# LANL-Bioinformatics/KWAGE

Hardware: AMD Instinct MI355X
Metric: G k-mer·sample bit-tests/sec (+ achieved HBM GB/s of the gather kernel in `roofline`) (higher is better)
Workload: dtype u32

## Files before the change

### kwage_amd/csrc/engine.hip

```cpp
#include <hip/hip_runtime.h>
#include <hip/hip_ext.h>

#include <algorithm>
#include <chrono>
#include <cmath>
#include <cstdio>
#include <cctype>
#include <cstring>
#include <new>
#include <string>
#include <thread>
#include <vector>

#include <unistd.h>

#include "host.hpp"
#include "engine_state.hpp"
#include "kernels.hpp"

using namespace kwage;


struct TuningName { const char *name; int64_t Tuning::*field; };
static const TuningName TUNING_NAMES[] = {
	{"walk", &Tuning::walk}, {"walk_min_rows", &Tuning::walk_min_rows}, {"walk_max_kib", &Tuning::walk_max_kib}, {"walk_min_kib", &Tuning::walk_min_kib}, {"walk_tile_kib", &Tuning::walk_tile_kib},
	 {"walk_waves", &Tuning::walk_waves}, {"walk_one_wg_per_cu", &Tuning::walk_one_wg_per_cu},
	{"walk_bands", &Tuning::walk_bands}, {"walk_bands_min_gib", &Tuning::walk_bands_min_gib},
	{"and_vec", &Tuning::and_vec}, {"and_wide", &Tuning::and_wide}, {"and_wide_min_kib", &Tuning::and_wide_min_kib}, {"narrow", &Tuning::narrow}, {"force_segs", &Tuning::force_segs},
	{"ee_refine", &Tuning::ee_refine}, {"refine_seg_rows", &Tuning::refine_seg_rows}, {"refine_min_rows", &Tuning::refine_min_rows}, {"refine_max_groups", &Tuning::refine_max_groups}, {"refine_unroll", &Tuning::refine_unroll}, {"refine_list_cap", &Tuning::refine_list_cap}, {"refine_static", &Tuning::refine_static}, {"screen_wpc", &Tuning::screen_wpc}, {"count_screen_wpc", &Tuning::count_screen_wpc}, {"count_screen_min_tiles", &Tuning::count_screen_min_tiles}, {"count_screen_check", &Tuning::count_screen_check}, {"count_trunc", &Tuning::count_trunc},
	{"count_walk", &Tuning::count_walk}, {"count_walk_wpc", &Tuning::count_walk_wpc}, {"count_walk_waves", &Tuning::count_walk_waves},
	{"count_walk_min_rows", &Tuning::count_walk_min_rows},
	{"hit_sort_host", &Tuning::hit_sort_host}, {"hit_copy_piece_kb", &Tuning::hit_copy_piece_kb}, {"shared_table_log2", &Tuning::shared_table_log2},
	{"ext_launch_events", &Tuning::ext_launch_events}, {"group_contiguous", &Tuning::group_contiguous}, {"group_placement_probe", &Tuning::group_placement_probe},
};

namespace kwage {

__global__ __launch_bounds__(KM_THREADS) void kmer_kernel(KmerArgs a)
{
	extern __shared__ __attribute__((aligned(16))) unsigned long long lds_tab[];
	__shared__ uint8_t codes[KM_THREADS + KWAGE_MAX_WORD_LEN];
	__shared__ uint32_t count, tile_base;

	const uint32_t q = a.chunk_q ? a.chunk_q[blockIdx.x] : blockIdx.x;
	const uint64_t t_begin = a.chunk_q ? a.chunk_t0[blockIdx.x] : 0;
	const uint64_t s0 = a.seq_off[q];
	const uint64_t len = a.seq_off[q + 1] - s0;
	const uint64_t npos = (len >= a.k) ? (len - a.k + 1) : 0;

	if(npos == 0){
		if(threadIdx.x == 0){ a.nkmer[q] = 0; a.qthr[q] = 0; }
		return;
	}

	if(a.shared_lg){
		kmer_body<false, false>(a, q, s0, len, 0, npos, a.g_tables, a.shared_lg, codes, &count, &tile_base);
		return;
	}
	const uint32_t lg = table_log2(npos);
	if((1ull << lg) <= a.lds_slots){
		kmer_body<true, false>(a, q, s0, len, 0, npos, lds_tab, lg, codes, &count, &tile_base);
	}
	else if(npos <= KM_CHUNK){
		kmer_body<false, false>(a, q, s0, len, 0, npos, a.g_tables + a.tab_off[q], lg, codes, &count, &tile_base);
	}
	else{
		kmer_body<false, true>(a, q, s0, len, t_begin, min(npos, t_begin + (uint64_t)KM_CHUNK), a.g_tables + a.tab_off[q], lg, codes, &count, &tile_base);
	}
}

__global__ __launch_bounds__(256) void kmer_finish_kernel(KmerArgs a, uint32_t n_queries)
{
	const uint32_t q = blockIdx.x*blockDim.x + threadIdx.x;
	if(q < n_queries){ a.qthr[q] = a.complete_match ? 0u : (uint32_t)__fmul_rn(a.threshold, (float)a.nkmer[q]); }
}

__global__ __launch_bounds__(256) void remap_rows_kernel(uint32_t *rows, const uint64_t *pos_off, const uint32_t *nkmer, uint32_t num_hash,
                                                         const uint32_t *map, uint32_t map_len, unsigned long long *missing, uint32_t wgs_per_query)
{
	const uint32_t q = blockIdx.x / wgs_per_query, part = blockIdx.x % wgs_per_query;
	uint32_t *rq = rows + pos_off[q]*num_hash;
	const uint64_t n = (uint64_t)nkmer[q]*num_hash;
	for(uint64_t e = (uint64_t)part*blockDim.x + threadIdx.x; e < n; e += (uint64_t)wgs_per_query*blockDim.x){
		const uint32_t r = rq[e];
		uint32_t lo = 0, hi = map_len;
		while(lo < hi){
			const uint32_t mid = lo + (hi - lo)/2;
			if(map[mid] < r){ lo = mid + 1; } else { hi = mid; }
		}
		if(lo < map_len && map[lo] == r){ rq[e] = lo; }
		else{ rq[e] = 0; atomicAdd(missing, 1ull); }
	}
}

__global__ __launch_bounds__(SEARCH_THREADS) void and_refine_emit_kernel(SearchArgs a, RefineArgs ra)
{
	constexpr int B = 4;
	__shared__ WaveHitBuf hit_bufs[SEARCH_THREADS/WAVE];
	WaveHitBuf *hbuf = &hit_bufs[threadIdx.x >> 6];
	WaveHitState hst;
	const uint32_t lane = threadIdx.x & (WAVE - 1), l = lane & 7u, g = lane >> 3;
	const uint32_t n_clusters = refine_list_end(ra, 0);
	const uint32_t gw = __builtin_amdgcn_readfirstlane(blockIdx.x*(blockDim.x/WAVE) + (threadIdx.x >> 6));
	const uint32_t nw = gridDim.x*(blockDim.x/WAVE);
	for(uint64_t c0 = gw; c0 < n_clusters; c0 += (uint64_t)B*nw){
		RefineCluster cl[B];
		u32x4 m[B];
#pragma unroll
		for(int k = 0; k < B; ++k){
			const uint64_t ci = c0 + (uint64_t)k*nw;
			cl[k].q = REFINE_NONE;
			if(ci < n_clusters){ cl[k] = ra.clusters[ci]; }
// ... 371 lines not shown
		case 10: launch_count_nh<10>(a, s, ge); break;
		case 14: launch_count_nh<14>(a, s, ge); break;
		case 20: launch_count_nh<20>(a, s, ge); break;
		default: launch_count_nh<32>(a, s, ge); break;
	}
}

template <int PLANES, int NH, bool TRUNC>
void launch_count_walk(const SearchArgs &a, const CountWalkArgs &wa, const RefineArgs &ra, const WalkShape &w, hipStream_t s, const StageEvents &ge)
{
	if(w.lds > 48*1024){ (void)hipFuncSetAttribute((const void*)count_walk_kernel<PLANES, NH, TRUNC>, hipFuncAttributeMaxDynamicSharedMemorySize, (int)w.lds); }
	KW_GATHER_LAUNCH(ge, true, !TRUNC, (count_walk_kernel<PLANES, NH, TRUNC>), dim3(w.wgs), dim3(w.wg_waves*WAVE), w.lds, s, a, wa, ra, a.rows, a.pos_off, a.nkmer, a.qthr);
}

template <int PLANES, bool TRUNC>
void launch_count_walk_nh(const SearchArgs &a, const CountWalkArgs &wa, const RefineArgs &ra, const WalkShape &w, hipStream_t s, const StageEvents &ge)
{
	switch(a.num_hash){
		case 1: launch_count_walk<PLANES, 1, TRUNC>(a, wa, ra, w, s, ge); break;
		case 2: launch_count_walk<PLANES, 2, TRUNC>(a, wa, ra, w, s, ge); break;
		case 3: launch_count_walk<PLANES, 3, TRUNC>(a, wa, ra, w, s, ge); break;
		case 4: launch_count_walk<PLANES, 4, TRUNC>(a, wa, ra, w, s, ge); break;
		default: launch_count_walk<PLANES, 5, TRUNC>(a, wa, ra, w, s, ge); break;
	}
}

template <bool TRUNC>
void launch_count_walk_planes(uint32_t planes, const SearchArgs &a, const CountWalkArgs &wa, const RefineArgs &ra, const WalkShape &w, hipStream_t s, const StageEvents &ge)
{
	switch(planes){
		case 7: launch_count_walk_nh<TRUNC ? 10 : 7, TRUNC>(a, wa, ra, w, s, ge); break;
		case 10: launch_count_walk_nh<10, TRUNC>(a, wa, ra, w, s, ge); break;
		case 14: launch_count_walk_nh<14, TRUNC>(a, wa, ra, w, s, ge); break;
		case 20: launch_count_walk_nh<20, TRUNC>(a, wa, ra, w, s, ge); break;
		default: launch_count_walk_nh<32, TRUNC>(a, wa, ra, w, s, ge); break;
	}
}

struct RefineSetup { RefineArgs ra; uint32_t refine_wgs, emit_wgs; };

int check_refine_units(uint32_t planes, int up)
{
	if(up == 14 && planes < 14){ return fail(KWAGE_ERR_STATE, "count refine: 14-plane units with %u counter planes", planes); }
	return KWAGE_OK;
}

void launch_count_refine_and_emit(uint32_t planes, int up, const SearchArgs &a, const RefineSetup &rs, hipStream_t gs, const StageEvents &ge)
{
	const dim3 block(SEARCH_THREADS);
#define KWAGE_CR_NH(N) case N: if(up == 7){ KW_GATHER_LAUNCH(ge, false, false, (count_refine_kernel<N, 7>), dim3(rs.refine_wgs), block, 0, gs, a, rs.ra); } \
		else{ KW_GATHER_LAUNCH(ge, false, false, (count_refine_kernel<N, 14>), dim3(rs.refine_wgs), block, 0, gs, a, rs.ra); } break;
	switch(std::min(a.num_hash, 5u)){ KWAGE_CR_NH(1) KWAGE_CR_NH(2) KWAGE_CR_NH(3) KWAGE_CR_NH(4) default: KWAGE_CR_NH(5) }
#undef KWAGE_CR_NH
#define KWAGE_CE_P(P) case P: if(up == 7){ KW_GATHER_LAUNCH(ge, false, true, (count_refine_emit_kernel<P, 7>), dim3(rs.emit_wgs), block, 0, gs, a, rs.ra); } \
		else{ KW_GATHER_LAUNCH(ge, false, true, (count_refine_emit_kernel<P, (P >= 14 ? 14 : 7)>), dim3(rs.emit_wgs), block, 0, gs, a, rs.ra); } break;
	switch(planes){ KWAGE_CE_P(7) KWAGE_CE_P(10) KWAGE_CE_P(14) KWAGE_CE_P(20) default: KWAGE_CE_P(32) }
#undef KWAGE_CE_P
}

template <int PLANES>
int launch_count_combine(const SearchArgs &a, uint32_t seg_planes, hipStream_t s, const StageEvents &ge)
{
	const size_t lds = (size_t)(COMBINE_WAVES/2)*PLANES*WAVE*16;
	if(lds > 48*1024){
		HIP_TRY(hipFuncSetAttribute((const void*)count_combine_kernel<PLANES>, hipFuncAttributeMaxDynamicSharedMemorySize, (int)lds));
	}
	KW_GATHER_LAUNCH(ge, false, true, (count_combine_kernel<PLANES>), dim3((a.units_per_row + WAVE - 1)/WAVE, a.n_queries), dim3(COMBINE_WAVES*WAVE), lds, s, a, seg_planes);
	return KWAGE_OK;
}

uint64_t max_segments(const SearchArgs &a, uint64_t max_segs) { return (a.n_queries > 65535) ? 1 : max_segs; }

int reserve_zeroed(DevBuf &buf, uint64_t bytes, hipStream_t s)
{
	if(bytes <= buf.cap){ return KWAGE_OK; }
	int rc = buf.reserve(bytes);
	if(rc){ return rc; }
	HIP_TRY(hipMemsetAsync(buf.p, 0, buf.cap, s));
	return KWAGE_OK;
}

int refine_setup(Slot *sl, const Tuning &tn, const SearchArgs &a, uint64_t total_rows, uint64_t max_rows, uint32_t max_seg, uint64_t item_bytes, uint64_t unit_bytes,
                 uint64_t tiles, uint64_t screen_waves, uint64_t ncu, hipStream_t gs, RefineSetup *out,
                 uint64_t exact_clusters = 0, uint64_t exact_items = 0, uint64_t exact_units = 0)
{
	int rc;
	RefineArgs &ra = out->ra;
	ra.seg_rows = (uint32_t)std::min<int64_t>(std::max<int64_t>(tn.refine_seg_rows, 8), max_seg);
	ra.seg_rows = (uint32_t)std::max<uint64_t>(ra.seg_rows, (max_rows + 65535)/65536);
	ra.min_rows = (uint32_t)std::max<int64_t>(tn.refine_min_rows, 1);
	ra.max_groups = (uint32_t)std::min<int64_t>(std::max<int64_t>(tn.refine_max_groups, 0), 16);
	uint64_t items = std::min<uint64_t>(std::max<uint64_t>(8ull*a.n_queries, 1u << 16), 1u << 20);
	items = std::max<uint64_t>(std::min<uint64_t>(items, (256ull << 20)/item_bytes), 1024);
	uint64_t units = std::min<uint64_t>(std::max<uint64_t>(32*total_rows/ra.seg_rows, 1u << 18), 1u << 25);
	if(unit_bytes){ units = std::max<uint64_t>(std::min<uint64_t>(units, (512ull << 20)/unit_bytes), 4096); }
	if(tn.refine_list_cap > 0){ items = units = (uint64_t)std::min<int64_t>(tn.refine_list_cap, 1 << 20); }
	uint64_t clusters = items;
	if(exact_units){ clusters = exact_clusters; items = exact_items; units = exact_units; }
	if(exact_units && tn.refine_list_cap > 0){ clusters = items = units = (uint64_t)std::min<int64_t>(tn.refine_list_cap, 1 << 20); }
	const uint64_t tiles_per_wave = (tiles + screen_waves - 1)/std::max<uint64_t>(screen_waves, 1);
	auto list = [&](uint64_t cap, uint64_t stat_max, uint64_t chunk_max) {
		RefineList ls;
		ls.cap = (uint32_t)cap;
		ls.stat = (tn.refine_static && !exact_units) ? (uint32_t)std::min<uint64_t>(stat_max, cap/2/std::max<uint64_t>(screen_waves, 1)) : 0u;
		ls.base = (uint32_t)(ls.stat*screen_waves);
		ls.chunk = exact_units ? 1u : (uint32_t)std::max<uint64_t>(1, std::min<uint64_t>(chunk_max, tiles_per_wave/4));
		return ls;
	};
	ra.lc = list(clusters, 32, 32);
	ra.li = list(items, 64, 64);
	ra.lu = list(units, 256, 256);
	if((rc = sl->ref_counters.reserve(8*sizeof(uint32_t)))){ return rc; }
	if((rc = sl->ref_clusters.reserve(clusters*sizeof(RefineCluster)))){ return rc; }
	if((rc = sl->ref_masks.reserve(items*item_bytes))){ return rc; }
	if((rc = sl->ref_units.reserve(units*sizeof(RefineUnit)))){ return rc; }
	if(unit_bytes && (rc = sl->ref_slab.reserve(units*unit_bytes))){ return rc; }
	ra.counters = (uint32_t*)sl->ref_counters.p;
	ra.clusters = (RefineCluster*)sl->ref_clusters.p;
	ra.masks = (uint32_t*)sl->ref_masks.p;
	ra.units = (RefineUnit*)sl->ref_units.p;
	ra.slab = (uint32_t*)sl->ref_slab.p;
	HIP_TRY(hipMemsetAsync(ra.counters, 0, 8*sizeof(uint32_t), gs));
	sl->ref_base[0] = ra.lc.base; sl->ref_base[1] = ra.li.base; sl->ref_base[2] = ra.lu.base;
	sl->ref_cap[0] = ra.lc.cap; sl->ref_cap[1] = ra.li.cap; sl->ref_cap[2] = ra.lu.cap;
	ra.queue_batch = (uint32_t)std::max<uint64_t>(1, std::min<uint64_t>(16, tiles/(8*std::max<uint64_t>(screen_waves, 1))));
	ra.check_every = (tn.count_screen_check == 16 || tn.count_screen_check == 32 || tn.count_screen_check == 64) ? (uint32_t)tn.count_screen_check : 8u;
	out->refine_wgs = (uint32_t)(ncu*8);
	out->emit_wgs = (uint32_t)(ncu*4);
	return KWAGE_OK;
}

uint32_t count_screen_blocks_per_cu(uint32_t planes, uint32_t nh)
{
	static int cache[3][5] = {};
	const int pi = (planes <= 7) ? 0 : (planes <= 10) ? 1 : 2, ni = (int)std::min(std::max(nh, 1u), 5u) - 1;
	if(cache[pi][ni] == 0){
		int nb = 0;
		hipError_t e = hipErrorUnknown;
#define KWAGE_OCC_NH(P, N) case N: e = hipOccupancyMaxActiveBlocksPerMultiprocessor(&nb, count_screen_kernel<P, N>, SEARCH_THREADS, 0); break;
#define KWAGE_OCC_P(I, P) case I: switch(ni + 1){ KWAGE_OCC_NH(P, 1) KWAGE_OCC_NH(P, 2) KWAGE_OCC_NH(P, 3) KWAGE_OCC_NH(P, 4) default: KWAGE_OCC_NH(P, 5) } break;
		switch(pi){ KWAGE_OCC_P(0, 7) KWAGE_OCC_P(1, 10) default: KWAGE_OCC_P(2, 14) }
#undef KWAGE_OCC_P
#undef KWAGE_OCC_NH
		if(e != hipSuccess || nb <= 0){ (void)hipGetLastError(); nb = 2; }
		cache[pi][ni] = nb;
	}
	return (uint32_t)cache[pi][ni];
}

int launch_search_stage(Slot *sl, kwage_group *g, kwage_batch *b, const KmerLayout *L, float threshold, uint32_t flags,
                        kwage_hit *d_hits, uint64_t cap, unsigned long long *hit_count, hipStream_t gs, const StageEvents &ge)
{
	const Tuning &tn = g->ctx->tune;
	const uint64_t ncu = (uint64_t)std::max(g->ctx->ncu, 1);
	SearchArgs a;
	a.db = g->d_bits;
	a.stride = g->stride;
	a.units_per_row = (uint32_t)(g->stride/16);
	a.valid = g->d_valid;
	a.rows = (const uint32_t*)sl->rows.p;
	a.pos_off = L->d_pos_off;
	a.nkmer = sl->d_nkmer;
	a.qthr = sl->d_qthr;
	a.num_hash = g->params.num_hash;
	a.n_queries = b->n;
	a.hits = d_hits;
	a.cap = cap;
	a.hit_count = hit_count;
	a.early_exit = (flags & KWAGE_SEARCH_EARLY_EXIT) ? 1 : 0;
	a.partial = nullptr;
	a.col_base = sl->col_base;
	a.runs = sl->n_runs ? (unsigned long long*)sl->runs.p : nullptr;
	a.runs_per_query = sl->runs_per_query;
	int rc;

	if(threshold == 1.0f){
		const uint64_t wide_tiles = (uint64_t)a.n_queries*((a.units_per_row + 4*WAVE - 1)/(4*WAVE));
		const bool wide_ok = tn.and_wide && !(flags & KWAGE_SEARCH_EARLY_EXIT) && wide_tiles >= 8*ncu;
		const bool wide_rows = wide_ok && a.units_per_row > (uint32_t)std::max<int64_t>(tn.and_wide_min_kib, 1)*WAVE;
		const AndCfg cfg = and_config(tn, a.units_per_row, wide_rows);
		a.chunks = (a.units_per_row + WAVE*cfg.vec - 1)/(WAVE*cfg.vec);
		choose_segments(a, L->max_pos, max_segments(a, 4096), tn.force_segs);
		if((uint64_t)a.n_queries*a.segs*a.chunks/4 + 1 > 0x7FFFFFFFull){ return fail(KWAGE_ERR_ARG, "batch too large for one launch"); }
		if(tn.narrow && a.segs == 1 && a.units_per_row <= 32 && a.n_queries >= 64){
			const uint32_t G = (a.units_per_row <= 4) ? 16 : (a.units_per_row <= 8) ? 8 : (a.units_per_row <= 16) ? 4 : 2;
			const uint64_t waves = ((uint64_t)a.n_queries + G - 1)/G;
			const dim3 grid((uint32_t)((waves + 3)/4)), block(SEARCH_THREADS);
			const int unroll = (waves < ncu*16) ? 16 : 8;
			snprintf(sl->kernel_name, sizeof(sl->kernel_name), "and_narrow_kernel<%u,%d>", G, unroll);
#define KWAGE_NARROW_CASE(GG) case GG: \
				if(unroll == 16){ KW_GATHER_LAUNCH(ge, true, true, (and_narrow_kernel<GG, 16>), grid, block, 0, gs, a); } \
				else{ KW_GATHER_LAUNCH(ge, true, true, (and_narrow_kernel<GG, 8>), grid, block, 0, gs, a); } break;
			switch(G){
				KWAGE_NARROW_CASE(16) KWAGE_NARROW_CASE(8) KWAGE_NARROW_CASE(4)
				default: KWAGE_NARROW_CASE(2)
			}
#undef KWAGE_NARROW_CASE
			HIP_TRY(hipGetLastError());
			return KWAGE_OK;
		}
		if(a.early_exit && tn.ee_refine && a.units_per_row >= WAVE && tn.force_segs <= 0){
			RefineSetup rs;
			const int vec = (a.units_per_row >= 4*WAVE) ? 2 : 1;
			a.segs = 1;
			a.chunks = (a.units_per_row + WAVE*vec - 1)/(WAVE*vec);
			const uint64_t tiles = (uint64_t)a.n_queries*a.chunks;
			const uint64_t screen_waves = (std::min<uint64_t>(tiles, ncu*(uint64_t)std::max<int64_t>(tn.screen_wpc, 1)) + 3)/4*4;
			if((rc = refine_setup(sl, tn, a, L->total_pos*a.num_hash, L->max_pos*a.num_hash, 1u << 20, 128, 0, tiles, screen_waves, ncu, gs, &rs))){ return rc; }
			const int unroll = (tn.refine_unroll == 16) ? 16 : 8;
			snprintf(sl->kernel_name, sizeof(sl->kernel_name), "and_screen_kernel<%d,8>+refine<%d>", vec, unroll);
			const dim3 grid((uint32_t)(screen_waves/4)), block(SEARCH_THREADS);
			if(vec == 2){ KW_GATHER_LAUNCH(ge, true, false, (and_screen_kernel<2, 8>), grid, block, 0, gs, a, rs.ra); }
			else{ KW_GATHER_LAUNCH(ge, true, false, (and_screen_kernel<1, 8>), grid, block, 0, gs, a, rs.ra); }
			if(unroll == 16){ KW_GATHER_LAUNCH(ge, false, false, (and_refine_kernel<16>), dim3(rs.refine_wgs), block, 0, gs, a, rs.ra); }
			else{ KW_GATHER_LAUNCH(ge, false, false, (and_refine_kernel<8>), dim3(rs.refine_wgs), block, 0, gs, a, rs.ra); }
			KW_GATHER_LAUNCH(ge, false, true, and_refine_emit_kernel, dim3(rs.emit_wgs), block, 0, gs, a, rs.ra);
			HIP_TRY(hipGetLastError());
			return KWAGE_OK;
		}
		const int walk_knob = (int)tn.walk;
		const uint64_t walk_min_rows = (tn.walk_min_rows >= 0) ? (uint64_t)tn.walk_min_rows : (uint64_t)WALK_MIN_ROWS_PER_WAVE*256*WALK_WAVES_PER_CU;
		const uint32_t kib = (a.units_per_row + WAVE - 1)/WAVE;
		const uint32_t walk_max_kib = (uint32_t)std::max<int64_t>(tn.walk_max_kib, 0);
		const uint32_t walk_tile = (uint32_t)std::min<int64_t>(std::max<int64_t>(tn.walk_tile_kib, 1), 16);
		const uint32_t coltiles = (kib + walk_tile - 1)/walk_tile, walk_ch = (kib + coltiles - 1)/coltiles;
		const bool walk_ee_ok = !a.early_exit;
		const uint64_t walk_slots = (uint64_t)coltiles*L->total_pos;
		const uint32_t walk_min_kib = (uint32_t)std::max<int64_t>(tn.walk_min_kib, 1);
		const int walk_unroll = (walk_ch <= 2) ? 8 : 4;
		if(walk_knob && walk_ee_ok && kib >= walk_min_kib && kib <= walk_max_kib && walk_slots*a.num_hash >= walk_min_rows && walk_slots > 0){
			const uint64_t chip_waves = ncu*WALK_WAVES_PER_CU;
			const uint64_t want_waves = (tn.walk_waves > 0) ? std::min<uint64_t>((uint64_t)tn.walk_waves, walk_slots)
				: std::max<uint64_t>(1, std::min<uint64_t>(chip_waves, walk_slots*a.num_hash/WALK_MIN_ROWS_PER_WAVE));
			const WalkShape shape = walk_shape(tn, want_waves, ncu);
			const uint32_t wgs = shape.wgs;
			const uint64_t waves = (uint64_t)wgs*shape.wg_waves;
			const uint64_t band_items = L->total_pos*a.num_hash;
			const bool big_enough = g->alloc_bytes >= ((uint64_t)std::max<int64_t>(tn.walk_bands_min_gib, 0) << 30);
			const uint32_t bands = !big_enough ? 0u : (tn.walk_bands < 0) ? (g->mixes_regions ? 3u : 0u) : (uint32_t)std::min<int64_t>(tn.walk_bands, BAND_MAX);
			if(bands >= 2 && coltiles == 1 && walk_ch >= 3 &&
			   (uint64_t)a.n_queries*16*1024 <= (256ull << 20) && band_items < 0x7FFFFFFFull){
				BandArgs ba;
				ba.bands = bands;
				ba.rows_per_band = (uint32_t)((g->nrows + bands - 1)/bands);
				if((rc = sl->band_rows.reserve(band_items*sizeof(uint32_t)))){ return rc; }
				if((rc = sl->band_loc.reserve((uint64_t)a.n_queries*(bands + 1)*sizeof(uint32_t)))){ return rc; }
				if((rc = reserve_zeroed(sl->band_or, (uint64_t)a.n_queries*16*1024, gs))){ return rc; }
				if((rc = reserve_zeroed(sl->band_state, (uint64_t)a.n_queries*sizeof(uint32_t), gs))){ return rc; }
				ba.orbuf = (uint32_t*)sl->band_or.p;
				ba.state = (uint32_t*)sl->band_state.p;
				uint32_t *loc = (uint32_t*)sl->band_loc.p, *rows2 = (uint32_t*)sl->band_rows.p;
				KW_GATHER_LAUNCH(ge, true, false, band_bucket_kernel, dim3(a.n_queries), dim3(256), 0, gs, a.rows, a.pos_off, a.nkmer, a.num_hash,
				                 ba.bands, ba.rows_per_band, loc, rows2);
				WalkArgs wb;
				wb.total_slots = walk_slots;
				wb.per_wave = (walk_slots + waves - 1)/waves;
				wb.coltiles = 1;
				wb.orbuf = nullptr; wb.done = nullptr;
				a.segs = 1;
				a.chunks = 1;
				snprintf(sl->kernel_name, sizeof(sl->kernel_name), "and_band_walk_kernel<%u,4>", walk_ch);
				const dim3 grid(wgs), block(shape.wg_waves*WAVE), fgrid((a.n_queries + 3)/4);
#define KWAGE_BAND_LAUNCH(CH, U) do { \
					if(shape.lds > 48*1024){ (void)hipFuncSetAttribute((const void*)and_band_walk_kernel<CH, U>, hipFuncAttributeMaxDynamicSharedMemorySize, (int)shape.lds); } \
					KW_GATHER_LAUNCH(ge, false, false, (and_band_walk_kernel<CH, U>), grid, block, shape.lds, gs, a, ba, wb, (const uint32_t*)rows2, (const uint32_t*)loc, a.pos_off, a.nkmer); \
					KW_GATHER_LAUNCH(ge, false, true, (and_band_finish_kernel<CH>), fgrid, dim3(256), 0, gs, a, ba, a.nkmer); } while(0)
#define KWAGE_BAND_CASE(CH) case CH: \
					KWAGE_BAND_LAUNCH(CH, 4); break;
				switch(walk_ch){
					KWAGE_BAND_CASE(3) KWAGE_BAND_CASE(4) KWAGE_BAND_CASE(5) KWAGE_BAND_CASE(6) KWAGE_BAND_CASE(7)
					KWAGE_BAND_CASE(8) KWAGE_BAND_CASE(9) KWAGE_BAND_CASE(10) KWAGE_BAND_CASE(11) KWAGE_BAND_CASE(12)
					KWAGE_BAND_CASE(13) KWAGE_BAND_CASE(14) KWAGE_BAND_CASE(15)
					default: KWAGE_BAND_CASE(16)
				}
#undef KWAGE_BAND_CASE
#undef KWAGE_BAND_LAUNCH
				HIP_TRY(hipGetLastError());
				return KWAGE_OK;
			}
			WalkArgs wa;
			wa.total_slots = walk_slots;
			wa.per_wave = (walk_slots + waves - 1)/waves;
			wa.coltiles = coltiles;
			if((rc = reserve_zeroed(sl->walk_or, waves*16*1024, gs))){ return rc; }
			if((rc = reserve_zeroed(sl->walk_done, waves*2*sizeof(uint32_t), gs))){ return rc; }
			wa.orbuf = (uint32_t*)sl->walk_or.p;
			wa.done = (uint32_t*)sl->walk_done.p;
			a.segs = 1;
			a.chunks = coltiles;
			snprintf(sl->kernel_name, sizeof(sl->kernel_name), "and_walk_kernel<%u,%d>", walk_ch, walk_unroll);
			const dim3 grid(wgs), block(shape.wg_waves*WAVE);
#define KWAGE_WALK_LAUNCH(...) do { \
				if(shape.lds > 48*1024){ (void)hipFuncSetAttribute((const void*)and_walk_kernel<__VA_ARGS__>, hipFuncAttributeMaxDynamicSharedMemorySize, (int)shape.lds); } \
				KW_GATHER_LAUNCH(ge, true, true, (and_walk_kernel<__VA_ARGS__>), grid, block, shape.lds, gs, a, wa, a.rows, a.pos_off, a.nkmer); } while(0)
#define KWAGE_WALK_CASE(CH) case CH: KWAGE_WALK_LAUNCH(CH, 4); break;
#define KWAGE_WALK_CASE8(CH) case CH: KWAGE_WALK_LAUNCH(CH, 8); break;
// ... 1076 lines not shown
```

### kwage_amd/csrc/engine_state.hpp

```cpp
#ifndef KWAGE_AMD_ENGINE_STATE_HPP
#define KWAGE_AMD_ENGINE_STATE_HPP

#include <hip/hip_runtime.h>

#include <algorithm>
#include <deque>
#include <memory>
#include <mutex>
#include <vector>

#include "internal.h"

#define HIP_TRY(expr)                                                                          \
	do {                                                                                       \
		hipError_t _e = (expr);                                                                \
		if(_e != hipSuccess){                                                                  \
			return fail(KWAGE_ERR_DEVICE, "%s failed: %s (%s:%d)", #expr, hipGetErrorString(_e), \
			            __FILE__, __LINE__);                                                   \
		}                                                                                      \
	} while(0)

struct kwage_group;
struct kwage_batch;
struct kwage_ctx;
// ... 149 lines not shown
	{
		if(!b.p){ return; }
		{
			std::lock_guard<std::mutex> lock(mu);
			uint64_t held = 0;
			for(const PinBuf &c : cached){ held += c.cap; }
			if(open && cached.size() < MAX_CACHED_BLOCKS && held + b.cap <= MAX_CACHED_BYTES){
				cached.push_back(b);
				b.p = nullptr; b.cap = 0;
				return;
			}
		}
		b.release();
	}
	void close()
	{
		std::lock_guard<std::mutex> lock(mu);
		open = false;
		for(PinBuf &c : cached){ c.release(); }
		cached.clear();
	}
};


struct Slot {
	hipStream_t stream = nullptr;
	hipEvent_t ev[4] = {nullptr, nullptr, nullptr, nullptr};
	hipEvent_t kmer_done = nullptr;
	hipEvent_t gather_done = nullptr;
	DevBuf rows, tables, partial;
	DevBuf result;
	uint64_t *d_counters = nullptr;
	uint32_t *d_nkmer = nullptr, *d_qthr = nullptr;
	kwage_hit *d_hits = nullptr;
	uint64_t hit_cap = 0, head_bytes = 0;
	PinBuf h_stage;
	DevBuf sort_scratch;
	DevBuf runs;
	uint64_t n_runs = 0;
	uint32_t runs_per_query = 0;
	bool busy = false;
	kwage_group *g = nullptr;
	kwage_batch *b = nullptr;
	const KmerLayout *lay = nullptr;
	float threshold = 1.0f;
	uint32_t flags = 0;
	uint32_t launches = 0;
	char kernel_name[64] = "";
	DevBuf walk_or, walk_done;
	DevBuf band_rows, band_loc, band_or, band_state;
	DevBuf cwalk_slab, cwalk_arrived;
	DevBuf ref_counters, ref_clusters, ref_masks, ref_units, ref_slab;
	DevBuf trunc_dev;
	PinBuf trunc_host;
	uint32_t ref_base[3] = {0, 0, 0}, ref_cap[3] = {0, 0, 0};
	uint64_t staged_hits = 0;
	kwage_hit *ext_hits = nullptr;
	uint64_t ext_cap = 0;
	uint64_t *ext_count = nullptr;
	bool append = false, append_reset = false;
	uint32_t col_base = 0;
};

struct Tuning {
	int64_t walk = 4;
	int64_t walk_min_rows = -1;
	int64_t walk_max_kib = 16;
	int64_t walk_tile_kib = 16;
	int64_t walk_min_kib = 2;
	int64_t walk_waves = 0;
	int64_t walk_one_wg_per_cu = 1;
	int64_t walk_bands = -1;
	int64_t walk_bands_min_gib = 48;
	int64_t and_vec = 0;
	int64_t and_wide_min_kib = 16;
	int64_t and_wide = 1;
	int64_t narrow = 1;
	int64_t force_segs = 0;
	int64_t ee_refine = 1;
	int64_t refine_seg_rows = 32;
	int64_t refine_min_rows = 32;
	int64_t refine_max_groups = 4;
	int64_t refine_unroll = 8;
	int64_t screen_wpc = 20;
	int64_t count_screen_wpc = 32;
	int64_t count_screen_min_tiles = 8192;
	int64_t count_trunc = 1;
	int64_t count_screen_check = 8;
	int64_t refine_static = 1;
	int64_t refine_list_cap = 0;
	int64_t count_walk = 1;
	int64_t count_walk_wpc = 8;
	int64_t count_walk_waves = 0;
	int64_t count_walk_min_rows = -1;
	int64_t hit_sort_host = 0;
	int64_t hit_copy_piece_kb = 0;
	int64_t ext_launch_events = 1;
	int64_t shared_table_log2 = 0;
	int64_t group_contiguous = 1;
	int64_t group_placement_probe = 1;
};

}

struct kwage_ctx {
	int device = -1;
	int ncu = 0;
	kwage::Tuning tune;
	hipStream_t stream = nullptr;
	hipStream_t gather_stream = nullptr;
	hipStream_t upload_stream = nullptr;
	kwage::Slot slot[2];
	kwage::DevBuf kmers;
	kwage::DevPool batch_pool;
	kwage::PinBuf load_pin[2];
	kwage::DevBuf load_dev[3];
	hipEvent_t load_done[3] = {nullptr, nullptr, nullptr};
	void *map_base = nullptr;
	size_t map_len = 0;
	hipEvent_t map_done = nullptr;
	struct LockedWindow { void *base; size_t len; hipEvent_t done; bool owns_event; };
	std::deque<LockedWindow> locked;
	std::vector<hipEvent_t> spare_events;
	volatile uint64_t *load_progress = nullptr;
	std::shared_ptr<kwage::PinnedPool> result_pool = std::make_shared<kwage::PinnedPool>();
	std::vector<int> numa_cpus;
	int numa_node = -1;
};

struct kwage_group {
	kwage_ctx *ctx = nullptr;
	kwage_params params{};
	uint64_t nrows = 0;
	uint64_t stride = 0;
	uint64_t next_byte = 0;
	uint64_t num_columns = 0;
	uint8_t *d_bits = nullptr;
	uint8_t *d_valid = nullptr;
	uint64_t alloc_bytes = 0;
	uint32_t placement_candidates = 0;
	double placement_kept_gbps = 0, placement_other_gbps = 0;
	double placement_windowed_gbps = 0;
	bool mixes_regions = false;
	std::vector<uint8_t> h_valid;
	bool finalized = false;
	double density = 0.25;
	double density_max = 1.0;
	std::vector<uint32_t> h_row_map;
	uint32_t *d_row_map = nullptr;
};

namespace kwage {

struct KmerLayout {
	uint32_t k = 0;
	uint64_t total_pos = 0;
	uint64_t max_pos = 0;
	uint64_t table_slots = 0;
	uint64_t *d_pos_off = nullptr;
	uint64_t *d_tab_off = nullptr;
	uint32_t *d_chunk_q = nullptr;
	uint64_t *d_chunk_t0 = nullptr;
	uint64_t n_chunks = 0;
	bool multi_chunk = false;
	std::vector<uint64_t> h_pos_off;
	DevPool *pool = nullptr;
// ... 68 lines not shown
```

### kwage_amd/csrc/kernels.hpp

```cpp
#ifndef KWAGE_AMD_KERNELS_HPP
#define KWAGE_AMD_KERNELS_HPP

#include <hip/hip_runtime.h>
#include <stdint.h>

#include "kwage_amd.h"
#include "kmer_device.hpp"

namespace kwage {

static constexpr int WAVE = 64;
static constexpr int KM_THREADS = 256;
static constexpr uint32_t KM_LDS_SLOTS = 4096;
static constexpr uint32_t KM_CHUNK = 1024;
static constexpr uint64_t KM_EMPTY = ~0ull;
static constexpr int SEARCH_THREADS = 256;


__device__ __forceinline__ uint32_t table_log2(uint64_t npos)
{
	uint32_t lg = 6;
	while((1ull << lg) < 2*npos){ ++lg; }
	return lg;
}
// ... 334 lines not shown
		if(k0 >= k1){ return; }
	}
	const uint32_t nrows = (k1 - k0)*a.num_hash;
	const uint32_t *rq = a.rows + (a.pos_off[q] + k0)*a.num_hash;

	uint32_t unit[VEC];
	bool live[VEC];
	u32x4 acc[VEC];
#pragma unroll
	for(int v = 0; v < VEC; ++v){
		const uint32_t u = c*(WAVE*VEC) + v*WAVE + lane;
		live[v] = (u < a.units_per_row);
		unit[v] = live[v] ? u : (a.units_per_row - 1);
		acc[v] = ~(u32x4)(0u);
	}

	uint32_t i = 0;
	bool dead = false;
	for(; i + UNROLL <= nrows; i += UNROLL){
		u32x4 x[UNROLL][VEC];
#pragma unroll
		for(int u = 0; u < UNROLL; ++u){
			const uint32_t r = rq[i + u];
			const u32x4 *p = reinterpret_cast<const u32x4*>(a.db + (uint64_t)r*a.stride);
#pragma unroll
			for(int v = 0; v < VEC; ++v){ x[u][v] = load16<NT>(p + unit[v]); }
		}
#pragma unroll
		for(int u = 0; u < UNROLL; ++u){
#pragma unroll
			for(int v = 0; v < VEC; ++v){ acc[v] &= x[u][v]; }
		}
		if(a.early_exit){
			bool nz = false;
#pragma unroll
			for(int v = 0; v < VEC; ++v){ nz |= ((acc[v].x | acc[v].y | acc[v].z | acc[v].w) != 0); }
			if(!__any(nz)){ dead = true; break; }
		}
	}
	for(; !dead && i < nrows; ++i){
		const uint32_t r = rq[i];
		const u32x4 *p = reinterpret_cast<const u32x4*>(a.db + (uint64_t)r*a.stride);
#pragma unroll
		for(int v = 0; v < VEC; ++v){ acc[v] &= load16<NT>(p + unit[v]); }
	}

#pragma unroll
	for(int v = 0; v < VEC; ++v){
		if(SEG){
			if(live[v]){
				uint32_t *m = a.partial + ((uint64_t)q*a.units_per_row + unit[v])*4;
#pragma unroll
				for(int d = 0; d < 4; ++d){
					if(acc[v][d] != ~0u){ atomicAnd(m + d, acc[v][d]); }
				}
			}
		}
		else{
			emit_mask_hits(a, q, unit[v], acc[v], n, (uint64_t)q*a.runs_per_query + c*VEC + v, live[v]);
		}
	}
}

struct RefineUnit { uint32_t item, r0, r1, unit0, rq_lo, rq_hi, q, pad; };
struct RefineCluster {
	uint32_t q, kstep_groups, first_item, n;
	uint32_t first_unit, nseg, pad0, pad1;
};
static constexpr uint32_t REFINE_NONE = 0xFFFFFFFFu;

struct RefineList { uint32_t cap, stat, base, chunk; };
struct RefineArgs {
	uint32_t *counters;
	RefineCluster *clusters;
	uint32_t *masks;
	RefineUnit *units;
	uint32_t *slab;
	RefineList lc, li, lu;
	uint32_t seg_rows;
	uint32_t min_rows;
	uint32_t max_groups;
	uint32_t queue_batch;
	uint32_t check_every;
};

__device__ __forceinline__ uint32_t group_bits(uint64_t lanes)
{
	uint32_t g = 0;
#pragma unroll
	for(int k = 0; k < 8; ++k){ g |= ((lanes >> (8*k)) & 0xFFull) ? (1u << k) : 0u; }
	return g;
}

__device__ __forceinline__ uint32_t nth_set_bit(uint32_t bits, uint32_t j)
{
	for(uint32_t k = 0; k < j; ++k){ bits &= bits - 1; }
	return __ffs(bits) - 1;
}

struct RefineChunk { uint32_t next = 0, end = 0; };

__device__ __forceinline__ void refine_none_clusters(const RefineArgs &ra, uint32_t from, uint32_t to)
{
	to = min(to, ra.lc.cap);
	for(uint32_t i = from + (threadIdx.x & (WAVE - 1)); i < to; i += WAVE){ ra.clusters[i].q = REFINE_NONE; }
}
__device__ __forceinline__ void refine_none_units(const RefineArgs &ra, uint32_t from, uint32_t to)
{
	to = min(to, ra.lu.cap);
	for(uint32_t i = from + (threadIdx.x & (WAVE - 1)); i < to; i += WAVE){ ra.units[i].item = REFINE_NONE; }
}

__device__ __forceinline__ uint32_t refine_take(const RefineArgs &ra, int which, RefineChunk &ch, uint32_t need)
{
	const RefineList &ls = (which == 0) ? ra.lc : (which == 1) ? ra.li : ra.lu;
	if(ch.end - ch.next < need){
		if(which == 0){ refine_none_clusters(ra, ch.next, ch.end); } else if(which == 2){ refine_none_units(ra, ch.next, ch.end); }
		ch.next = ch.end = 0;
		if((uint64_t)ls.base + __hip_atomic_load(ra.counters + which, __ATOMIC_RELAXED, __HIP_MEMORY_SCOPE_AGENT) >= ls.cap){ return REFINE_NONE; }
		const uint32_t want = max(need, ls.chunk);
		uint32_t r = 0;
		if((threadIdx.x & (WAVE - 1)) == 0){ r = atomicAdd(ra.counters + which, want); }
		const uint64_t at = (uint64_t)ls.base + __builtin_amdgcn_readfirstlane(r);
		if(at + want > ls.cap){
			if(at < ls.cap){
				if(which == 0){ refine_none_clusters(ra, (uint32_t)at, ls.cap); } else if(which == 2){ refine_none_units(ra, (uint32_t)at, ls.cap); }
			}
			return REFINE_NONE;
		}
		ch.next = (uint32_t)at;
		ch.end = (uint32_t)at + want;
	}
	const uint32_t at = ch.next;
	ch.next += need;
	return at;
}

__device__ __forceinline__ uint32_t refine_list_end(const RefineArgs &ra, int which)
{
	const RefineList &ls = (which == 0) ? ra.lc : (which == 1) ? ra.li : ra.lu;
	return (uint32_t)min((uint64_t)ls.base + ra.counters[which], (uint64_t)ls.cap);
}

template <int VEC, int UNROLL>
__global__ __launch_bounds__(SEARCH_THREADS) void and_screen_kernel(SearchArgs a, RefineArgs ra)
{
	const uint32_t lane = threadIdx.x & (WAVE - 1);
	const uint64_t n_tiles = (uint64_t)a.n_queries*a.chunks;
	const uint32_t n_waves = gridDim.x*(blockDim.x/WAVE);
	const uint32_t gw = __builtin_amdgcn_readfirstlane(blockIdx.x*(blockDim.x/WAVE) + (threadIdx.x >> 6));
	__shared__ WaveHitBuf hit_bufs[SEARCH_THREADS/WAVE];
	WaveHitBuf *hbuf = &hit_bufs[threadIdx.x >> 6];
	WaveHitState hst;
	RefineChunk cc, ci, cu;
	cc.next = gw*ra.lc.stat; cc.end = cc.next + ra.lc.stat;
	ci.next = gw*ra.li.stat; ci.end = ci.next + ra.li.stat;
	cu.next = gw*ra.lu.stat; cu.end = cu.next + ra.lu.stat;
	bool lists_full = false;
	for(uint64_t tile = gw; tile < n_tiles; tile += n_waves){
		const uint32_t q = __builtin_amdgcn_readfirstlane((uint32_t)(tile / a.chunks));
		const uint32_t c = __builtin_amdgcn_readfirstlane((uint32_t)(tile % a.chunks));
		const uint32_t n = a.nkmer[q];
		if(n == 0){ continue; }
		const uint32_t nrows = n*a.num_hash;
		const uint64_t rq_off = a.pos_off[q]*a.num_hash;
		const uint32_t *rq = a.rows + rq_off;

		uint32_t unit[VEC];
		u32x4 acc[VEC];
#pragma unroll
		for(int v = 0; v < VEC; ++v){
			const uint32_t u = c*(WAVE*VEC) + v*WAVE + lane;
			const bool live = (u < a.units_per_row);
			unit[v] = live ? u : (a.units_per_row - 1);
			acc[v] = live ? reinterpret_cast<const u32x4*>(a.valid)[u] : (u32x4)(0u);
		}

		bool may_hand_over = !lists_full, gone = false;
		uint32_t i = 0;
		for(; i + UNROLL <= nrows; i += UNROLL){
			u32x4 x[UNROLL][VEC];
#pragma unroll
			for(int u = 0; u < UNROLL; ++u){
				const uint32_t r = rq[i + u];
				const u32x4 *p = reinterpret_cast<const u32x4*>(a.db + (uint64_t)r*a.stride);
#pragma unroll
				for(int v = 0; v < VEC; ++v){ x[u][v] = load16<true>(p + unit[v]); }
			}
#pragma unroll
			for(int u = 0; u < UNROLL; ++u){
#pragma unroll
				for(int v = 0; v < VEC; ++v){ acc[v] &= x[u][v]; }
			}
			uint32_t gb[VEC], ngroups = 0;
#pragma unroll
			for(int v = 0; v < VEC; ++v){
				gb[v] = group_bits(__ballot((acc[v].x | acc[v].y | acc[v].z | acc[v].w) != 0));
				ngroups += __popc(gb[v]);
			}
			if(ngroups == 0){ gone = true; break; }
			const uint32_t done = i + UNROLL;
			if(may_hand_over && ngroups <= ra.max_groups && nrows - done >= ra.min_rows && (done >= 2*UNROLL || nrows < 4*ra.seg_rows)){
				may_hand_over = false;
				const uint32_t nseg = (nrows - done + ra.seg_rows - 1)/ra.seg_rows;
				uint32_t nc = 0;
#pragma unroll
				for(int v = 0; v < VEC; ++v){ nc += gb[v] ? 1u : 0u; }
				const uint32_t nu = ngroups*nseg;
				const uint32_t c0 = refine_take(ra, 0, cc, nc);
				const uint32_t i0 = (c0 != REFINE_NONE) ? refine_take(ra, 1, ci, ngroups) : REFINE_NONE;
				const uint32_t u0 = (i0 != REFINE_NONE) ? refine_take(ra, 2, cu, nu) : REFINE_NONE;
				if(u0 == REFINE_NONE){
					if(c0 != REFINE_NONE){ refine_none_clusters(ra, c0, c0 + nc); }
					lists_full = true;
					continue;
				}
				uint32_t cidx = c0, ii = i0, all_groups = 0;
#pragma unroll
				for(int v = 0; v < VEC; ++v){
					all_groups |= gb[v] << (8*v);
					if(!gb[v]){ continue; }
					if(lane == 0){
						RefineCluster cl; cl.q = q; cl.kstep_groups = ((c*VEC + v) << 8) | gb[v]; cl.first_item = ii; cl.n = n;
						cl.first_unit = 0; cl.nseg = 0; cl.pad0 = 0; cl.pad1 = 0;
						ra.clusters[cidx] = cl;
					}
					const uint32_t k = lane >> 3;
					if((gb[v] >> k) & 1u){
						const uint32_t it = ii + __popc(gb[v] & ((1u << k) - 1u));
						reinterpret_cast<u32x4*>(ra.masks)[(uint64_t)it*8 + (lane & 7u)] = acc[v];
					}
					++cidx;
					ii += __popc(gb[v]);
				}
				for(uint32_t e = lane; e < nu; e += WAVE){
					const uint32_t j = e / nseg, sg = e % nseg;
					const uint32_t gpos = nth_set_bit(all_groups, j);
					RefineUnit un;
					un.item = i0 + j;
					un.r0 = done + sg*ra.seg_rows;
					un.r1 = min(nrows, un.r0 + ra.seg_rows);
					un.unit0 = c*(WAVE*VEC) + gpos*8u;
					un.rq_lo = (uint32_t)rq_off; un.rq_hi = (uint32_t)(rq_off >> 32);
					un.q = q; un.pad = 0;
					ra.units[u0 + e] = un;
				}
				gone = true;
				break;
			}
		}
		if(gone){ continue; }
		for(; i < nrows; ++i){
			const uint32_t r = rq[i];
			const u32x4 *p = reinterpret_cast<const u32x4*>(a.db + (uint64_t)r*a.stride);
#pragma unroll
			for(int v = 0; v < VEC; ++v){ acc[v] &= load16<true>(p + unit[v]); }
		}
#pragma unroll
		for(int v = 0; v < VEC; ++v){
			emit_masked_hits_buffered(a, hbuf, hst, q, unit[v], acc[v], n, (uint64_t)q*a.runs_per_query + c*VEC + v);
		}
	}
	wave_hits_flush(a, hbuf, hst);
	refine_none_clusters(ra, cc.next, cc.end);
	refine_none_units(ra, cu.next, cu.end);
}

template <int UNROLL>
__global__ __launch_bounds__(SEARCH_THREADS) void and_refine_kernel(SearchArgs a, RefineArgs ra)
{
	static_assert(UNROLL == 8 || UNROLL == 16, "eight or sixteen rows in flight");
	const uint32_t lane = threadIdx.x & (WAVE - 1), l = lane & 7u, sh = lane & ~7u;
	const uint32_t n_units = refine_list_end(ra, 2);
	const uint64_t gw = (uint64_t)blockIdx.x*(blockDim.x/WAVE) + (threadIdx.x >> 6);
	const uint64_t step = (uint64_t)gridDim.x*(blockDim.x/WAVE)*8;
	for(uint64_t base = gw*8; base < n_units; base += step){
		const uint64_t u = base + (lane >> 3);
		RefineUnit un;
		un.item = REFINE_NONE;
		if(u < n_units){ un = ra.units[u]; }
		bool on = (un.item != REFINE_NONE);
		uint32_t *M = ra.masks;
		u32x4 m = (u32x4)(0u);
		if(on){
			M = ra.masks + ((uint64_t)un.item*8 + l)*4;
#pragma unroll
			for(int d = 0; d < 4; ++d){ m[d] = __hip_atomic_load(M + d, __ATOMIC_RELAXED, __HIP_MEMORY_SCOPE_AGENT); }
		}
		on = on && (((uint32_t)(__ballot((m.x | m.y | m.z | m.w) != 0) >> sh) & 0xFFu) != 0);
		if(on){
			const uint32_t *rq = a.rows + (((uint64_t)un.rq_hi << 32) | un.rq_lo);
			const u32x4 *col = reinterpret_cast<const u32x4*>(a.db) + (un.unit0 + l);
			u32x4 acc = ~(u32x4)(0u);
			bool alive = true;
			for(uint32_t b = un.r0; alive && b < un.r1; b += 64){
				uint32_t idx[8];
#pragma unroll
				for(int k = 0; k < 8; ++k){ idx[k] = rq[min(b + 8u*k + l, un.r1 - 1)]; }
#pragma unroll
				for(int k = 0; k < 8; k += UNROLL/8){
					if(b + 8u*k >= un.r1){ break; }
					u32x4 x[UNROLL];
#pragma unroll
					for(int j = 0; j < UNROLL; ++j){
						const uint32_t r = __shfl(idx[k + j/8], sh + (j & 7));
						x[j] = load16<true>(reinterpret_cast<const u32x4*>(reinterpret_cast<const uint8_t*>(col) + (uint64_t)r*a.stride));
					}
#pragma unroll
					for(int j = 0; j < UNROLL; ++j){ acc &= x[j]; }
					if((((uint32_t)(__ballot((acc.x | acc.y | acc.z | acc.w) != 0) >> sh)) & 0xFFu) == 0){ alive = false; break; }
				}
			}
#pragma unroll
			for(int d = 0; d < 4; ++d){
				if(m[d] & ~acc[d]){ __hip_atomic_fetch_and(M + d, acc[d], __ATOMIC_RELAXED, __HIP_MEMORY_SCOPE_AGENT); }
			}
		}
	}
}


static constexpr int WALK_WG_WAVES = 8;
static constexpr uint32_t WALK_DEAD = 1u;
static constexpr uint32_t WALK_DIRTY = 2u;

struct WalkArgs {
	uint64_t total_slots;
	uint64_t per_wave;
	uint32_t coltiles;
	uint32_t *orbuf;
	uint32_t *done;
};

template <int CH, int UNROLL>
__global__ __launch_bounds__(WALK_WG_WAVES*WAVE) __attribute__((amdgpu_waves_per_eu(2, 2))) void and_walk_kernel(SearchArgs a, WalkArgs wa, const uint32_t *__restrict__ rows,
// ... 1026 lines not shown
```

Measured before the change: 52170.

## Add in-wave narrow refinement in AND screen kernel and skip refine lists when small

When only a few 8-lane groups of a tile remain live and few rows are left, the screen kernel now finishes those groups itself. Each wave splits the remaining rows across its lanes, loads many rows in flight per lane, and combines results with cross-lane AND reductions, instead of handing work to the separate refine and emit kernels. If every query's row count fits under the in-wave threshold, the refine lists are sized to zero and the refine and emit launches are skipped entirely. This removes list-management atomics, extra kernel launches and the underused tail loop. In exchange the serialized per-group loop can leave a wave running long on tiles with many rows.

```diff
diff --git a/kwage_amd/csrc/engine.hip b/kwage_amd/csrc/engine.hip
--- a/kwage_amd/csrc/engine.hip
+++ b/kwage_amd/csrc/engine.hip
@@ -27,7 +27,7 @@
 	 {"walk_waves", &Tuning::walk_waves}, {"walk_one_wg_per_cu", &Tuning::walk_one_wg_per_cu},
 	{"walk_bands", &Tuning::walk_bands}, {"walk_bands_min_gib", &Tuning::walk_bands_min_gib},
 	{"and_vec", &Tuning::and_vec}, {"and_wide", &Tuning::and_wide}, {"and_wide_min_kib", &Tuning::and_wide_min_kib}, {"narrow", &Tuning::narrow}, {"force_segs", &Tuning::force_segs},
-	{"ee_refine", &Tuning::ee_refine}, {"refine_seg_rows", &Tuning::refine_seg_rows}, {"refine_min_rows", &Tuning::refine_min_rows}, {"refine_max_groups", &Tuning::refine_max_groups}, {"refine_unroll", &Tuning::refine_unroll}, {"refine_list_cap", &Tuning::refine_list_cap}, {"refine_static", &Tuning::refine_static}, {"screen_wpc", &Tuning::screen_wpc}, {"count_screen_wpc", &Tuning::count_screen_wpc}, {"count_screen_min_tiles", &Tuning::count_screen_min_tiles}, {"count_screen_check", &Tuning::count_screen_check}, {"count_trunc", &Tuning::count_trunc},
+	{"ee_refine", &Tuning::ee_refine}, {"refine_seg_rows", &Tuning::refine_seg_rows}, {"refine_min_rows", &Tuning::refine_min_rows}, {"refine_max_groups", &Tuning::refine_max_groups}, {"refine_unroll", &Tuning::refine_unroll}, {"refine_inwave_rows", &Tuning::refine_inwave_rows}, {"refine_inwave_first", &Tuning::refine_inwave_first}, {"refine_inwave_fallback", &Tuning::refine_inwave_fallback},{"refine_list_cap", &Tuning::refine_list_cap}, {"refine_static", &Tuning::refine_static}, {"screen_wpc", &Tuning::screen_wpc}, {"count_screen_wpc", &Tuning::count_screen_wpc}, {"count_screen_min_tiles", &Tuning::count_screen_min_tiles}, {"count_screen_check", &Tuning::count_screen_check}, {"count_trunc", &Tuning::count_trunc},
 	{"count_walk", &Tuning::count_walk}, {"count_walk_wpc", &Tuning::count_walk_wpc}, {"count_walk_waves", &Tuning::count_walk_waves},
 	{"count_walk_min_rows", &Tuning::count_walk_min_rows},
 	{"hit_sort_host", &Tuning::hit_sort_host}, {"hit_copy_piece_kb", &Tuning::hit_copy_piece_kb}, {"shared_table_log2", &Tuning::shared_table_log2},
@@ -565,7 +565,7 @@
 
 int refine_setup(Slot *sl, const Tuning &tn, const SearchArgs &a, uint64_t total_rows, uint64_t max_rows, uint32_t max_seg, uint64_t item_bytes, uint64_t unit_bytes,
                  uint64_t tiles, uint64_t screen_waves, uint64_t ncu, hipStream_t gs, RefineSetup *out,
-                 uint64_t exact_clusters = 0, uint64_t exact_items = 0, uint64_t exact_units = 0)
+                 uint64_t exact_clusters = 0, uint64_t exact_items = 0, uint64_t exact_units = 0, bool no_lists = false)
 {
 	int rc;
 	RefineArgs &ra = out->ra;
@@ -581,6 +581,7 @@
 	uint64_t clusters = items;
 	if(exact_units){ clusters = exact_clusters; items = exact_items; units = exact_units; }
 	if(exact_units && tn.refine_list_cap > 0){ clusters = items = units = (uint64_t)std::min<int64_t>(tn.refine_list_cap, 1 << 20); }
+	if(no_lists){ clusters = items = units = 0; }
 	const uint64_t tiles_per_wave = (tiles + screen_waves - 1)/std::max<uint64_t>(screen_waves, 1);
 	auto list = [&](uint64_t cap, uint64_t stat_max, uint64_t chunk_max) {
 		RefineList ls;
@@ -593,7 +594,7 @@
 	ra.lc = list(clusters, 32, 32);
 	ra.li = list(items, 64, 64);
 	ra.lu = list(units, 256, 256);
-	if((rc = sl->ref_counters.reserve(8*sizeof(uint32_t)))){ return rc; }
+	if((rc = reserve_zeroed(sl->ref_counters, 8*sizeof(uint32_t), gs))){ return rc; }
 	if((rc = sl->ref_clusters.reserve(clusters*sizeof(RefineCluster)))){ return rc; }
 	if((rc = sl->ref_masks.reserve(items*item_bytes))){ return rc; }
 	if((rc = sl->ref_units.reserve(units*sizeof(RefineUnit)))){ return rc; }
@@ -603,10 +604,12 @@
 	ra.masks = (uint32_t*)sl->ref_masks.p;
 	ra.units = (RefineUnit*)sl->ref_units.p;
 	ra.slab = (uint32_t*)sl->ref_slab.p;
-	HIP_TRY(hipMemsetAsync(ra.counters, 0, 8*sizeof(uint32_t), gs));
+	if(!no_lists){ HIP_TRY(hipMemsetAsync(ra.counters, 0, 8*sizeof(uint32_t), gs)); }
 	sl->ref_base[0] = ra.lc.base; sl->ref_base[1] = ra.li.base; sl->ref_base[2] = ra.lu.base;
 	sl->ref_cap[0] = ra.lc.cap; sl->ref_cap[1] = ra.li.cap; sl->ref_cap[2] = ra.lu.cap;
 	ra.queue_batch = (uint32_t)std::max<uint64_t>(1, std::min<uint64_t>(16, tiles/(8*std::max<uint64_t>(screen_waves, 1))));
+	ra.inwave_rows = 0;
+	ra.inwave_flags = 0;
 	ra.check_every = (tn.count_screen_check == 16 || tn.count_screen_check == 32 || tn.count_screen_check == 64) ? (uint32_t)tn.count_screen_check : 8u;
 	out->refine_wgs = (uint32_t)(ncu*8);
 	out->emit_wgs = (uint32_t)(ncu*4);
@@ -689,12 +692,20 @@
 			a.chunks = (a.units_per_row + WAVE*vec - 1)/(WAVE*vec);
 			const uint64_t tiles = (uint64_t)a.n_queries*a.chunks;
 			const uint64_t screen_waves = (std::min<uint64_t>(tiles, ncu*(uint64_t)std::max<int64_t>(tn.screen_wpc, 1)) + 3)/4*4;
-			if((rc = refine_setup(sl, tn, a, L->total_pos*a.num_hash, L->max_pos*a.num_hash, 1u << 20, 128, 0, tiles, screen_waves, ncu, gs, &rs))){ return rc; }
+			const uint64_t inwave_rows = (uint64_t)std::min<int64_t>(std::max<int64_t>(tn.refine_inwave_rows, 0), 0xFFFFFFFFll);
+			const bool screen_only = inwave_rows > 0 && L->max_pos*a.num_hash <= inwave_rows;
+			if((rc = refine_setup(sl, tn, a, L->total_pos*a.num_hash, L->max_pos*a.num_hash, 1u << 20, 128, 0, tiles, screen_waves, ncu, gs, &rs, 0, 0, 0, screen_only))){ return rc; }
+			rs.ra.inwave_rows = (uint32_t)inwave_rows;
+			rs.ra.inwave_flags = (tn.refine_inwave_first ? INWAVE_FIRST : 0u) | (tn.refine_inwave_fallback ? INWAVE_FALLBACK : 0u);
 			const int unroll = (tn.refine_unroll == 16) ? 16 : 8;
 			snprintf(sl->kernel_name, sizeof(sl->kernel_name), "and_screen_kernel<%d,8>+refine<%d>", vec, unroll);
 			const dim3 grid((uint32_t)(screen_waves/4)), block(SEARCH_THREADS);
-			if(vec == 2){ KW_GATHER_LAUNCH(ge, true, false, (and_screen_kernel<2, 8>), grid, block, 0, gs, a, rs.ra); }
-			else{ KW_GATHER_LAUNCH(ge, true, false, (and_screen_kernel<1, 8>), grid, block, 0, gs, a, rs.ra); }
+			if(vec == 2){ KW_GATHER_LAUNCH(ge, true, screen_only, (and_screen_kernel<2, 8>), grid, block, 0, gs, a, rs.ra); }
+			else{ KW_GATHER_LAUNCH(ge, true, screen_only, (and_screen_kernel<1, 8>), grid, block, 0, gs, a, rs.ra); }
+			if(screen_only){
+				HIP_TRY(hipGetLastError());
+				return KWAGE_OK;
+			}
 			if(unroll == 16){ KW_GATHER_LAUNCH(ge, false, false, (and_refine_kernel<16>), dim3(rs.refine_wgs), block, 0, gs, a, rs.ra); }
 			else{ KW_GATHER_LAUNCH(ge, false, false, (and_refine_kernel<8>), dim3(rs.refine_wgs), block, 0, gs, a, rs.ra); }
 			KW_GATHER_LAUNCH(ge, false, true, and_refine_emit_kernel, dim3(rs.emit_wgs), block, 0, gs, a, rs.ra);
diff --git a/kwage_amd/csrc/engine_state.hpp b/kwage_amd/csrc/engine_state.hpp
--- a/kwage_amd/csrc/engine_state.hpp
+++ b/kwage_amd/csrc/engine_state.hpp
@@ -255,6 +255,9 @@
 	int64_t refine_min_rows = 32;
 	int64_t refine_max_groups = 4;
 	int64_t refine_unroll = 8;
+	int64_t refine_inwave_rows = 1024;
+	int64_t refine_inwave_first = 1;
+	int64_t refine_inwave_fallback = 1;
 	int64_t screen_wpc = 20;
 	int64_t count_screen_wpc = 32;
 	int64_t count_screen_min_tiles = 8192;
diff --git a/kwage_amd/csrc/kernels.hpp b/kwage_amd/csrc/kernels.hpp
--- a/kwage_amd/csrc/kernels.hpp
+++ b/kwage_amd/csrc/kernels.hpp
@@ -440,7 +440,12 @@
 	uint32_t max_groups;
 	uint32_t queue_batch;
 	uint32_t check_every;
+	uint32_t inwave_rows;
+	uint32_t inwave_flags;
 };
+static constexpr uint32_t INWAVE_FIRST = 1u;
+static constexpr uint32_t INWAVE_FALLBACK = 2u;
+static constexpr int INWAVE_LOADS = 8;
 
 __device__ __forceinline__ uint32_t group_bits(uint64_t lanes)
 {
@@ -498,6 +503,53 @@
 {
 	const RefineList &ls = (which == 0) ? ra.lc : (which == 1) ? ra.li : ra.lu;
 	return (uint32_t)min((uint64_t)ls.base + ra.counters[which], (uint64_t)ls.cap);
+}
+
+template <int D, int T>
+__device__ __forceinline__ void and_inwave_loads(const uint8_t *col, uint64_t stride, const uint32_t (&idx)[D/8], u32x4 (&x)[D])
+{
+	if constexpr(T < D){
+		const uint32_t r = (uint32_t)__builtin_amdgcn_ds_swizzle((int)idx[T >> 3], 0x18 | ((T & 7) << 5));
+		x[T] = load16<true>(reinterpret_cast<const u32x4*>(col + (uint64_t)r*stride));
+		and_inwave_loads<D, T + 1>(col, stride, idx, x);
+	}
+}
+
+template <int D>
+__device__ __forceinline__ u32x4 and_inwave_group(const SearchArgs &a, const uint32_t *rq, uint32_t r0, uint32_t nrows, uint32_t unit0, u32x4 gm)
+{
+	static_assert(D == 8 || D == 16, "eight or sixteen rows in flight per lane");
+	constexpr int NI = D/8;
+	uint32_t lane = threadIdx.x & (WAVE - 1);
+	asm volatile("" : "+v"(lane));
+	const uint32_t l = lane & 7u;
+	const u32x4 *col = reinterpret_cast<const u32x4*>(a.db) + min(unit0 + l, a.units_per_row - 1);
+	uint32_t idx[NI];
+#pragma unroll
+	for(int k = 0; k < NI; ++k){ idx[k] = rq[min(r0 + 64u*k + lane, nrows - 1)]; }
+	for(uint32_t b = r0; b < nrows; b += 8u*D){
+		u32x4 x[D];
+		and_inwave_loads<D, 0>(reinterpret_cast<const uint8_t*>(col), a.stride, idx, x);
+		uint32_t nxt[NI];
+#pragma unroll
+		for(int k = 0; k < NI; ++k){ nxt[k] = rq[min(b + 8u*D + 64u*k + lane, nrows - 1)]; }
+		u32x4 p = x[0];
+#pragma unroll
+		for(int t = 1; t < D; ++t){ p &= x[t]; }
+#pragma unroll
+		for(int d = 8; d < WAVE; d <<= 1){
+#pragma unroll
+			for(int e = 0; e < 4; ++e){ p[e] &= __shfl_xor(p[e], d); }
+		}
+		gm &= p;
+#pragma unroll
+		for(int k = 0; k < NI; ++k){
+			asm volatile("" : "+v"(nxt[k]));
+			idx[k] = nxt[k];
+		}
+		if(!__any((gm.x | gm.y | gm.z | gm.w) != 0)){ break; }
+	}
+	return gm;
 }
 
 template <int VEC, int UNROLL>
@@ -534,7 +586,7 @@
 			acc[v] = live ? reinterpret_cast<const u32x4*>(a.valid)[u] : (u32x4)(0u);
 		}
 
-		bool may_hand_over = !lists_full, gone = false;
+		bool may_hand_over = !lists_full, gone = false, narrowed = false;
 		uint32_t i = 0;
 		for(; i + UNROLL <= nrows; i += UNROLL){
 			u32x4 x[UNROLL][VEC];
@@ -558,6 +610,23 @@
 			}
 			if(ngroups == 0){ gone = true; break; }
 			const uint32_t done = i + UNROLL;
+			const bool inwave_ok = ra.inwave_rows != 0 && ngroups <= ra.max_groups && done < nrows && (done >= 2*UNROLL || (ra.inwave_flags & INWAVE_FIRST));
+			if(inwave_ok && (nrows - done <= ra.inwave_rows || (!may_hand_over && (ra.inwave_flags & INWAVE_FALLBACK)))){
+#pragma unroll
+				for(int v = 0; v < VEC; ++v){
+					for(uint32_t bits = gb[v]; bits; bits &= bits - 1){
+						const uint32_t k = __ffs(bits) - 1;
+						u32x4 gm;
+#pragma unroll
+						for(int e = 0; e < 4; ++e){ gm[e] = __shfl(acc[v][e], (int)(8*k + (lane & 7u))); }
+						const uint32_t unit0 = c*(WAVE*VEC) + v*WAVE + 8*k;
+						gm = and_inwave_group<INWAVE_LOADS>(a, rq, done, nrows, unit0, gm);
+						if((lane >> 3) == k){ acc[v] = gm; }
+					}
+				}
+				narrowed = true;
+				break;
+			}
 			if(may_hand_over && ngroups <= ra.max_groups && nrows - done >= ra.min_rows && (done >= 2*UNROLL || nrows < 4*ra.seg_rows)){
 				may_hand_over = false;
 				const uint32_t nseg = (nrows - done + ra.seg_rows - 1)/ra.seg_rows;
@@ -608,7 +677,7 @@
 			}
 		}
 		if(gone){ continue; }
-		for(; i < nrows; ++i){
+		for(; !narrowed && i < nrows; ++i){
 			const uint32_t r = rq[i];
 			const u32x4 *p = reinterpret_cast<const u32x4*>(a.db + (uint64_t)r*a.stride);
 #pragma unroll
```

Result: no change. 52170 (median of 5 runs) (+0.0%).
